# phymhan/pc-gan

Hardware: AMD Instinct MI355X
Metric: images/sec (G+D step) 128x128 bs32 per GPU (higher is better)
Workload: dtype f32; 1 GPU; wsgan_emb UTKFace-shaped 128x128 bs32/GPU fp32: 9-block ResnetGenerator + 3-layer PatchGAN + ResNet-18 Elo encoder@224 + AlexNet IP@224, full optimize_parameters(); global_batch=32, parallelism=dp1

## Files before the change

include/pcgan_hip.h:

```cpp
#ifndef PCGAN_HIP_H
#define PCGAN_HIP_H

#include <stddef.h>
#include <stdint.h>

#ifdef __cplusplus
extern "C" {
#endif

typedef void* pcgan_stream_t;

const char* pcgan_last_error(void);
int pcgan_version(void);
int pcgan_device_info(int* cu_count, char* arch, int arch_len);

typedef struct {
    int N, C, H, W;
    int K, R, S;
    int stride, pad, pad_mode;
    int P, Q;
    int dtype;
} pcgan_conv_desc;

enum { PCGAN_ACT_NONE = 0, PCGAN_ACT_RELU = 1, PCGAN_ACT_LRELU = 2, PCGAN_ACT_TANH = 3, PCGAN_ACT_SIGMOID = 4 };
// ... 203 lines not shown
    int stride, pad_h, pad_w;
    int P, Q;
    int k_off, K_total;
    int dtype;
} pcgan_iconv_desc;
int pcgan_iconv_supported(const pcgan_iconv_desc* d);
size_t pcgan_iconv_packed_bytes(const pcgan_iconv_desc* d);
int pcgan_iconv_pack(const pcgan_iconv_desc* d, int pool_expand, const float* w, const float* gamma, const float* beta, const float* mean,
                     const float* var, float eps, void* packed, pcgan_stream_t s);
int pcgan_iconv_fwd(const pcgan_iconv_desc* d, const void* x, const void* packed, void* y, int relu, pcgan_stream_t s);
int pcgan_maxpool_slice_fwd(const void* x, void* y, int N, int C, int H, int W, int k, int stride, int P, int Q, int k_off, int K_total,
                            int dtype, pcgan_stream_t s);
int pcgan_inception_prep(const void* x, void* y, int N, int C, int H, int W, int OH, int OW, const float* scale, const float* shift,
                         int dtype, pcgan_stream_t s);

int pcgan_linear_softmax_fwd(const void* x, const float* w, const float* b, void* logits, void* probs, int N, int C, int K, int dtype,
                             pcgan_stream_t s);

int pcgan_set_nonfinite_counter(unsigned int* dev_word);
int pcgan_set_option(const char* key, int value);
int pcgan_get_option(const char* key, int* value);
int pcgan_timer_enable(int capacity);
int pcgan_timer_read(int kind, float* ms, int cap);
#define PCGAN_IGEMM_LAUNCH_INFO 7
#define PCGAN_IGEMM_HGEMM_F16X2 1
#define PCGAN_IGEMM_HGEMM_BF16 2
#define PCGAN_IGEMM_IGEMM2_CG16 3
#define PCGAN_IGEMM_IGEMM2_CG4 4
#define PCGAN_IGEMM_GENERIC 5
#define PCGAN_IGEMM_SMALLM 6
int pcgan_igemm_last_launch(int* info, int n);

#ifdef __cplusplus
}
#endif
#endif
```

pc-gan_amd/csrc/capi.hip:

```cpp
#include "common.h"
#include <stdarg.h>
#include <atomic>
#include <mutex>
#include <vector>

namespace pcgan {
static thread_local char g_err[512] = "";
void set_error(const char* fmt, ...) {
    va_list ap;
    va_start(ap, fmt);
    vsnprintf(g_err, sizeof(g_err), fmt, ap);
    va_end(ap);
}
}

namespace pcgan {
namespace {
struct TimerKind {
    std::vector<hipEvent_t> start, stop;
    int used = 0;
};
std::mutex g_timer_mu;
std::atomic<int> g_timer_on{0};
TimerKind g_timer[TIMER_KINDS];
// ... 49 lines not shown
    }
    std::lock_guard<std::mutex> lk(g_timer_mu);
    TimerKind& t = g_timer[kind];
    int n = 0;
    for (int i = 0; i < t.used && n < cap; ++i) {
        if (hipEventSynchronize(t.stop[i]) != hipSuccess) continue;
        float v = 0.f;
        if (hipEventElapsedTime(&v, t.start[i], t.stop[i]) == hipSuccess) ms[n++] = v;
    }
    t.used = 0;
    return n;
}

namespace pcgan {
static std::atomic<unsigned*> g_nonfinite{nullptr};
unsigned* nonfinite_counter() { return g_nonfinite.load(std::memory_order_relaxed); }
}
extern "C" int pcgan_set_nonfinite_counter(unsigned int* dev_word) {
    pcgan::g_nonfinite.store(dev_word);
    return 0;
}

namespace pcgan {
static const char* const g_opt_names[OPT_COUNT] = {"bsplit_halo", "wgrad_gen", "wgrad_padcopy", "wgrad_cw", "hgemm_bf16", "wgd_look", "wgrad_direct", "hgemm_tile", "hgemm_ks", "wgrad_rowring"};
static std::atomic<int> g_opt[OPT_COUNT] = {{1}, {1}, {0}, {0}, {1}, {3}, {0}, {0}, {0}, {1}};
int option(int id) { return (id >= 0 && id < OPT_COUNT) ? g_opt[id].load(std::memory_order_relaxed) : 0; }
static int option_index(const char* key) {
    for (int i = 0; key && i < OPT_COUNT; ++i)
        if (strcmp(key, g_opt_names[i]) == 0) return i;
    return -1;
}
}
extern "C" int pcgan_set_option(const char* key, int value) {
    using namespace pcgan;
    const int i = option_index(key);
    PCGAN_CHECK(i >= 0, "set_option: unknown option '%s' (bsplit_halo, wgrad_gen, wgrad_padcopy, wgrad_cw, hgemm_bf16, wgd_look, wgrad_direct, hgemm_tile, hgemm_ks, wgrad_rowring)", key ? key : "(null)");
    PCGAN_CHECK(i != OPT_WGRAD_CW || value == 0 || value == 128 || value == 256, "set_option: wgrad_cw takes 0 (default), 128 or 256, got %d", value);
    PCGAN_CHECK(i != OPT_HGEMM_TILE || value == 0 || value == 128128 || value == 128064 || value == 64128 || value == 64064,
                "set_option: hgemm_tile takes 0 (heuristic) or BM * 1000 + BP with BM, BP in {64, 128}, got %d", value);
    PCGAN_CHECK(i != OPT_HGEMM_KS || (value >= 0 && value <= 8), "set_option: hgemm_ks takes 0 (heuristic) .. 8, got %d", value);
    g_opt[i].store(value);
    return 0;
}
extern "C" int pcgan_get_option(const char* key, int* value) {
    using namespace pcgan;
    const int i = option_index(key);
    PCGAN_CHECK(i >= 0 && value, "get_option: unknown option or null output");
    *value = g_opt[i].load();
    return 0;
}

extern "C" const char* pcgan_last_error(void) { return pcgan::g_err; }
extern "C" int pcgan_version(void) { return 100; }

extern "C" int pcgan_device_info(int* cu_count, char* arch, int arch_len) {
    hipDeviceProp_t prop;
    hipError_t e = hipGetDeviceProperties(&prop, 0);
    if (e != hipSuccess) {
        pcgan::set_error("hipGetDeviceProperties failed: %s", hipGetErrorString(e));
// ... 10 lines not shown
```

pc-gan_amd/csrc/common.h:

```cpp
#pragma once
#include <hip/hip_runtime.h>
#include <stdint.h>
#include <stdio.h>
#include <string.h>
#include "../../include/pcgan_hip.h"

namespace pcgan {

void set_error(const char* fmt, ...);

#define PCGAN_CHECK(cond, ...)                \
    do {                                      \
        if (!(cond)) {                        \
            pcgan::set_error(__VA_ARGS__);    \
            return 1;                         \
        }                                     \
    } while (0)

#define PCGAN_LAUNCH_CHECK()                                                      \
    do {                                                                          \
        hipError_t e__ = hipGetLastError();                                       \
        if (e__ != hipSuccess) {                                                  \
            pcgan::set_error("%s:%d launch failed: %s", __FILE__, __LINE__,       \
                             hipGetErrorString(e__));                             \
            return 2;                                                             \
        }                                                                         \
    } while (0)

enum { TIMER_RES_FWD = 0, TIMER_RES_DGRAD = 1, TIMER_RES_WGRAD = 2, TIMER_RES_WGRAD_MAIN = 3, TIMER_KINDS = 4 };
struct TimerScope {
    int kind, slot;
    hipStream_t st;
    TimerScope(int kind, hipStream_t st);
    ~TimerScope();
};

static inline int timer_kind_res(const pcgan_conv_desc* d, int kind) {
    return (d && d->K == 256 && d->C == 256 && d->R == 3 && d->S == 3 && d->stride == 1 && d->pad_mode == 1 && d->pad == 1) ? kind : -1;
}

enum { OPT_BSPLIT_HALO = 0, OPT_WGRAD_GEN = 1, OPT_WGRAD_PADCOPY = 2, OPT_WGRAD_CW = 3, OPT_HGEMM_BF16 = 4, OPT_WGD_LOOK = 5, OPT_WGRAD_DIRECT = 6, OPT_HGEMM_TILE = 7, OPT_HGEMM_KS = 8, OPT_WGRAD_ROWRING = 9, OPT_COUNT = 10 };
int option(int id);

unsigned* nonfinite_counter();
int launch_wgd_reduce(const float* part, float* dw, const float* scales, int splits, int K, int C, int accumulate, hipStream_t st);
__device__ __forceinline__ bool is_nonfinite(float v) { return (__float_as_uint(v) & 0x7f800000u) == 0x7f800000u; }
__device__ __forceinline__ void report_nonfinite(unsigned* counter, bool bad) {
    if (counter != nullptr && __builtin_amdgcn_ballot_w64(bad) != 0ull && (threadIdx.x & 63) == 0) atomicAdd(counter, 1u);
}

int launch_weight_row_absmax(const float* w, int K, int C, int T, int by_c, float* out, hipStream_t st);

int launch_reflect_fold(const void* padded, void* dx, int NC, int H, int W, int pad, int dtype, hipStream_t st);

static inline int ilog2_exact(int v) {
    int l = 0;
    while ((1 << l) < v) ++l;
    return ((1 << l) == v) ? l : -1;
}
static inline size_t align_up(size_t v, size_t a) { return (v + a - 1) / a * a; }

__device__ __forceinline__ float act_apply(float v, int act, float slope) {
    switch (act) {
        case PCGAN_ACT_RELU: return v > 0.f ? v : 0.f;
// ... 127 lines not shown
```

pc-gan_amd/csrc/hgemm.hip:

```cpp
#include "igemm.h"

namespace pcgan {

typedef _Float16 f16x8 __attribute__((ext_vector_type(8)));
typedef _Float16 f16x4 __attribute__((ext_vector_type(4)));

typedef __bf16 bf16x8v __attribute__((ext_vector_type(8)));
typedef __bf16 bf16x4v __attribute__((ext_vector_type(4)));

template <int MODE, int BM, int BP, typename TA>
__global__ void __launch_bounds__(256) hgemm_kernel(IgemmArgs a) {
    static_assert(MODE == MODE_FWD_ZERO || MODE == MODE_FWD_REFLECT || MODE == MODE_BWD, "forward and plain data gradient");
    constexpr bool HALF = sizeof(TA) == 2;
    constexpr int NP = HALF ? 1 : 2;
    constexpr unsigned ES = sizeof(TA);
    constexpr int WM = (BM == 128 || (BM == 64 && BP == 64)) ? 2 : 1;
    constexpr int WP = 4 / WM;
    constexpr int WMT = BM / WM, WPT = BP / WP;
    constexpr int MI = WMT / 32, PJ = WPT / 32;
    constexpr int KPT = BP / 16;
    constexpr int ACH = BM * 4 / 256;
    constexpr int TROWS = NTAP_FWD + 1;
    constexpr int AH = BM + 8;
    __shared__ __attribute__((aligned(16))) f16x8 As[2][NP][2 * AH];
    __shared__ __attribute__((aligned(16))) f16x8 Bs[2][NP][2 * BP];
    __shared__ unsigned offT[TROWS][BP];
    __shared__ __attribute__((aligned(16))) float biasS[BM];
    __shared__ __attribute__((aligned(16))) float iswS[BM];

    const int nMt = (a.M + BM - 1) / BM;
    const int mt = blockIdx.x % nMt;
    int pt = blockIdx.x / nMt;
    int phase = 0;
    while (phase + 1 < a.nphase && pt >= a.tstart[phase + 1]) ++phase;
    pt -= a.tstart[phase];
    const PhaseArgs& P = a.ph[phase];
    const int tid = threadIdx.x;
    const int lane = tid & 63, lo = lane & 31, hi = lane >> 5;
    const int wave = __builtin_amdgcn_readfirstlane(tid >> 6);
    const int wm = wave / WP, wp = wave % WP;
    const int Ptot = P.Ptot, Kp = P.Kp;
    const int m0 = mt * BM, p0 = pt * BP;
    const int ph_nS = P.nS;
    const int T = P.nR * ph_nS;
    const int HgWg4 = a.Hg * a.Wg * (int)ES;
    const __amdgpu_buffer_rsrc_t rX = make_rsrc(a.X, a.x_bytes);
    const __amdgpu_buffer_rsrc_t rA = make_rsrc(P.A, (unsigned)a.M * (unsigned)Kp * 4u);

    float sx = 1.f;
    const int pl = tid % BP;
    {
        const int pg = p0 + pl;
        const bool pvalid = pg < Ptot;
        int gn = 0, py = 0, px = 0;
        if (pvalid) pix_coord(a, P, pg, gn, py, px);
        const unsigned vbase = (unsigned)gn * (unsigned)a.Cg * (unsigned)(a.Hg * a.Wg);
        for (int t = tid / BP; t <= T; t += 256 / BP) {
            const int ri = t / ph_nS, sj = t - ri * ph_nS;
            const int r = P.r0 + ri * a.tstep, sxx = P.s0 + sj * a.tstep;
            const bool live = pvalid && t < T;
            const unsigned y = axis_entry<MODE>(py, py + a.pad, true, r, a.Hg, a.sl, a.pad);
            const unsigned x = axis_entry<MODE>(px, px + a.pad, true, sxx, a.Wg, a.sl, a.pad);
            offT[t][pl] = (live && y != 0xffffffffu && x != 0xffffffffu) ? (vbase + y * (unsigned)a.Wg + x) * ES : OOB;
        }
    }
    const int ksub = __builtin_amdgcn_readfirstlane(tid / BP);
    __syncthreads();

    const int nst_all = Kp >> 4;
    const int nst_per = a.ksplit > 1 ? (nst_all + a.ksplit - 1) / a.ksplit : nst_all;
    const int st_begin = a.ksplit > 1 ? (int)blockIdx.z * nst_per : 0;
    const int st_end = st_begin + nst_per < nst_all ? st_begin + nst_per : nst_all;
    const int nst_here = st_end > st_begin ? st_end - st_begin : 0;

    int it_tap, it_c, it_k0, it_left = nst_here;
    {
        const int cc0 = st_begin / T;
        it_tap = st_begin - cc0 * T;
        it_c = cc0 * 16;
        it_k0 = st_begin * 16;
    }
    unsigned a_base[ACH];
#pragma unroll
    for (int j = 0; j < ACH; ++j) {
        const int q = tid + 256 * j;
        const int row = q >> 2, kc = (q & 3) * 4;
        a_base[j] = (m0 + row < a.M) ? (unsigned)((m0 + row) * Kp + kc) * 4u : OOB;
    }
    struct Stage {
        u32x4 av[ACH];
        unsigned bv[KPT];
    };
    auto load = [&](Stage& r) {
        const bool live = it_left > 0;
        const unsigned vo = offT[live ? it_tap : T][pl];
        const unsigned so = (unsigned)((it_c + ksub * KPT) * HgWg4);
#pragma unroll
        for (int j = 0; j < ACH; ++j) r.av[j] = __builtin_amdgcn_raw_buffer_load_b128(rA, live ? a_base[j] : OOB, (unsigned)it_k0 * 4u, 0);
#pragma unroll
        for (int i = 0; i < KPT; ++i) {
            if constexpr (HALF) r.bv[i] = (unsigned)__builtin_amdgcn_raw_buffer_load_b16(rX, vo, so + (unsigned)(i * HgWg4), 0);
            else r.bv[i] = __builtin_amdgcn_raw_buffer_load_b32(rX, vo, so + (unsigned)(i * HgWg4), 0);
        }
        --it_left;
        const int t1 = it_tap + 1;
        const bool wr = t1 == T;
        it_tap = wr ? 0 : t1;
        it_c += wr ? 16 : 0;
        it_k0 += 16;
    };
    auto stash = [&](const Stage& r, int buf) {
        if constexpr (HALF) {
#pragma unroll
            for (int j = 0; j < ACH; ++j) {
                const int q = tid + 256 * j;
                const int row = q >> 2, kc = (q & 3) * 4;
                bf16x4v h;
#pragma unroll
                for (int e = 0; e < 4; ++e) h[e] = (__bf16)__uint_as_float(r.av[j][e]);
                *reinterpret_cast<bf16x4v*>(reinterpret_cast<__bf16*>(&As[buf][0][(kc >> 3) * AH + row]) + (kc & 4)) = h;
            }
            typedef unsigned short usK __attribute__((ext_vector_type(KPT)));
            usK v;
#pragma unroll
            for (int e = 0; e < KPT; ++e) v[e] = (unsigned short)r.bv[e];
            if constexpr (KPT == 8) *reinterpret_cast<usK*>(&Bs[buf][0][ksub * BP + pl]) = v;
            else *reinterpret_cast<usK*>(reinterpret_cast<unsigned short*>(&Bs[buf][0][(ksub >> 1) * BP + pl]) + (ksub & 1) * 4) = v;
            return;
        }
#pragma unroll
        for (int j = 0; j < ACH; ++j) {
            const int q = tid + 256 * j;
            const int row = q >> 2, kc = (q & 3) * 4;
            typedef unsigned u32x2 __attribute__((ext_vector_type(2)));
            u32x2 h, l;
            h[0] = r.av[j][0]; h[1] = r.av[j][1];
            l[0] = r.av[j][2]; l[1] = r.av[j][3];
            _Float16* d0 = reinterpret_cast<_Float16*>(&As[buf][0][(kc >> 3) * AH + row]) + (kc & 4);
            _Float16* d1 = reinterpret_cast<_Float16*>(&As[buf][NP - 1][(kc >> 3) * AH + row]) + (kc & 4);
            *reinterpret_cast<u32x2*>(d0) = h;
            *reinterpret_cast<u32x2*>(d1) = l;
        }
        if constexpr (KPT == 8) {
            f16x8 h, l;
#pragma unroll
            for (int e = 0; e < 8; ++e) {
                _Float16 x, y;
                split2h(__uint_as_float(r.bv[e]) * sx, x, y);
                h[e] = x;
                l[e] = y;
            }
            Bs[buf][0][ksub * BP + pl] = h;
            Bs[buf][NP - 1][ksub * BP + pl] = l;
        } else {
            f16x4 h, l;
#pragma unroll
            for (int e = 0; e < 4; ++e) {
                _Float16 x, y;
                split2h(__uint_as_float(r.bv[e]) * sx, x, y);
                h[e] = x;
                l[e] = y;
            }
            *reinterpret_cast<f16x4*>(reinterpret_cast<_Float16*>(&Bs[buf][0][(ksub >> 1) * BP + pl]) + (ksub & 1) * 4) = h;
            *reinterpret_cast<f16x4*>(reinterpret_cast<_Float16*>(&Bs[buf][NP - 1][(ksub >> 1) * BP + pl]) + (ksub & 1) * 4) = l;
        }
    };

    f32x16 acc[MI][PJ];
#pragma unroll
    for (int i = 0; i < MI; ++i)
#pragma unroll
        for (int j = 0; j < PJ; ++j)
#pragma unroll
            for (int r = 0; r < 16; ++r) acc[i][j][r] = 0.f;
    struct Operands {
        f16x8 A[NP][MI], B[NP][PJ];
    };
    auto fetch = [&](Operands& o, int buf) {
#pragma unroll
        for (int p = 0; p < NP; ++p) {
#pragma unroll
            for (int i = 0; i < MI; ++i) o.A[p][i] = As[buf][p][hi * AH + wm * WMT + i * 32 + lo];
#pragma unroll
            for (int j = 0; j < PJ; ++j) o.B[p][j] = Bs[buf][p][hi * BP + wp * WPT + j * 32 + lo];
        }
    };
    auto mma = [&](const Operands& o) {
        if constexpr (HALF) {
#pragma unroll
            for (int i = 0; i < MI; ++i)
#pragma unroll
                for (int j = 0; j < PJ; ++j)
                    acc[i][j] = __builtin_amdgcn_mfma_f32_32x32x16_bf16(__builtin_bit_cast(bf16x8v, o.A[0][i]), __builtin_bit_cast(bf16x8v, o.B[0][j]),
                                                                         acc[i][j], 0, 0, 0);
            return;
        }
        constexpr int PA[3] = {NP - 1, 0, 0}, PB[3] = {0, NP - 1, 0};
#pragma unroll
        for (int q = 0; q < 3; ++q)
#pragma unroll
            for (int i = 0; i < MI; ++i)
#pragma unroll
                for (int j = 0; j < PJ; ++j)
                    acc[i][j] = __builtin_amdgcn_mfma_f32_32x32x16_f16(o.A[PA[q]][i], o.B[PB[q]][j], acc[i][j], 0, 0, 0);
    };
    auto interleave = [&]() {
        constexpr int NM = (HALF ? 1 : 3) * MI * PJ, NRD = NP * (MI + PJ);
#pragma unroll
        for (int q = 0; q < NM; ++q) {
            __builtin_amdgcn_sched_group_barrier(0x008, 1, 0);
            __builtin_amdgcn_sched_group_barrier(0x100, (NRD + NM - 1) / NM, 0);
            __builtin_amdgcn_sched_group_barrier(0x002, 48 / NM + 1, 0);
            __builtin_amdgcn_sched_group_barrier(0x200, 1, 0);
            __builtin_amdgcn_sched_group_barrier(0x020, (ACH + KPT + NM - 1) / NM, 0);
        }
    };

    Stage rg[2];
    if (nst_here > 0) {
        load(rg[0]);
        load(rg[1]);
    }
    if constexpr (!HALF) {
        const float m = thread_max_of_partials(a.x_amax, a.x_namax, tid, 256);
        sx = pow2_scale(block_max(m, biasS));
        if (tid < BM) iswS[tid] = m0 + tid < a.M ? 1.f / pow2_scale(a.w_amax[m0 + tid]) : 1.f;
        __syncthreads();
    }
    if (tid < BM) biasS[tid] = (a.bias != nullptr && m0 + tid < a.M) ? a.bias[m0 + tid] : 0.f;
    if (nst_here == 0) __syncthreads();
    if (nst_here > 0) {
        Operands op[2];
        stash(rg[0], 0);
        __syncthreads();
        load(rg[0]);
        fetch(op[0], 0);
        stash(rg[1], 1);
        __syncthreads();
        load(rg[1]);
        const int nst2 = (nst_here + 1) & ~1;
        for (int s = 0; s < nst2; s += 2) {
#pragma unroll
            for (int t = 0; t < 2; ++t) {
                fetch(op[t ^ 1], t ^ 1);
                mma(op[t]);
                stash(rg[t], t);
                load(rg[t]);
                interleave();
                __builtin_amdgcn_sched_barrier(0);
                __syncthreads();
                __builtin_amdgcn_sched_barrier(0);
            }
        }
    }

    const float isx = 1.f / sx;
    const int YhYw = a.Yh * a.Yw;
    bool bad = false;
    if constexpr (!HALF) {
#pragma unroll
        for (int j = 0; j < PJ; ++j)
#pragma unroll
            for (int i = 0; i < MI; ++i)
#pragma unroll
                for (int r = 0; r < 16; ++r) bad |= is_nonfinite(acc[i][j][r]);
        report_nonfinite(a.ovf, bad);
    }
#pragma unroll
    for (int j = 0; j < PJ; ++j) {
        const int pix = p0 + wp * WPT + j * 32 + lo;
        if (pix >= Ptot) continue;
        int n, oy, ox;
// ... 1 lines not shown
        if (a.ksplit > 1) {
            float* Yp = a.Ypart + ((size_t)blockIdx.z * a.N + n) * a.M * YhYw + oy * a.Yw + ox;
#pragma unroll
            for (int i = 0; i < MI; ++i)
#pragma unroll
                for (int r = 0; r < 16; ++r) {
                    const int ml = wm * WMT + i * 32 + (r & 3) + 8 * (r >> 2) + 4 * hi;
                    const int m = m0 + ml;
                    if (m < a.M) Yp[(size_t)m * YhYw] = (acc[i][j][r] * isx) * (HALF ? 1.f : iswS[ml]);
                }
            continue;
        }
        TA* Yp = (TA*)a.Y + (size_t)n * a.M * YhYw + oy * a.Yw + ox;
#pragma unroll
        for (int i = 0; i < MI; ++i)
#pragma unroll
            for (int r = 0; r < 16; ++r) {
                const int ml = wm * WMT + i * 32 + (r & 3) + 8 * (r >> 2) + 4 * hi;
                if (m0 + ml < a.M) st1(Yp + (size_t)(m0 + ml) * YhYw, act_apply((acc[i][j][r] * isx) * (HALF ? 1.f : iswS[ml]) + biasS[ml], a.act, a.slope));
            }
    }
}

template <int MODE>
static void launch_mode(const IgemmArgs& a, int bm, int bp, dim3 grid2, hipStream_t st) {
    if (bm == 128 && bp == 128) LAUNCH_TA(a.dtype, hgemm_kernel, grid2, a, MODE, 128, 128);
    else if (bm == 128) LAUNCH_TA(a.dtype, hgemm_kernel, grid2, a, MODE, 128, 64);
    else if (bp == 128) LAUNCH_TA(a.dtype, hgemm_kernel, grid2, a, MODE, 64, 128);
    else LAUNCH_TA(a.dtype, hgemm_kernel, grid2, a, MODE, 64, 64);
}
int launch_hgemm(int mode, const IgemmArgs& a, int bm, int bp, dim3 grid2, hipStream_t st) {
    switch (mode) {
        case MODE_FWD_ZERO: launch_mode<MODE_FWD_ZERO>(a, bm, bp, grid2, st); break;
        case MODE_FWD_REFLECT: launch_mode<MODE_FWD_REFLECT>(a, bm, bp, grid2, st); break;
        case MODE_BWD: launch_mode<MODE_BWD>(a, bm, bp, grid2, st); break;
        default: PCGAN_CHECK(false, "hgemm: no kernel for mode %d", mode);
    }
    PCGAN_LAUNCH_CHECK();
    return 0;
}

}

using namespace pcgan;

__global__ void __launch_bounds__(256) hgemm_presplit_kernel(float* __restrict__ A, int M, int Kp4, const float* __restrict__ rowmax) {
    const size_t n4 = (size_t)M * Kp4;
    for (size_t i = (size_t)blockIdx.x * 256 + threadIdx.x; i < n4; i += (size_t)gridDim.x * 256) {
        const float s = pow2_scale(rowmax[i / Kp4]);
        const float4 v = reinterpret_cast<const float4*>(A)[i];
        f16x4 h, l;
        _Float16 x, y;
        split2h(v.x * s, x, y); h[0] = x; l[0] = y;
        split2h(v.y * s, x, y); h[1] = x; l[1] = y;
// ... 13 lines not shown
```

pc-gan_amd/csrc/igemm.h:

```cpp
#pragma once
#include "common.h"
#include <type_traits>

namespace pcgan {

typedef float f32x16 __attribute__((ext_vector_type(16)));

enum { MODE_FWD_ZERO = 0, MODE_FWD_REFLECT = 1, MODE_BWD = 2, MODE_BWD_REFLECT = 3 };

typedef unsigned int u32x4 __attribute__((ext_vector_type(4)));
static constexpr unsigned OOB = 0x80000000u;

__device__ __forceinline__ __amdgpu_buffer_rsrc_t make_rsrc(const void* p, unsigned bytes) {
    return __builtin_amdgcn_make_buffer_rsrc(const_cast<void*>(p), 0, (int)bytes, 0x00020000);
}
__device__ __forceinline__ float ld_b32(__amdgpu_buffer_rsrc_t r, unsigned voff, unsigned soff) {
    return __uint_as_float(__builtin_amdgcn_raw_buffer_load_b32(r, voff, soff, 0));
}
__device__ __forceinline__ float4 ld_b128(__amdgpu_buffer_rsrc_t r, unsigned voff) {
    const u32x4 v = __builtin_amdgcn_raw_buffer_load_b128(r, voff, 0, 0);
    return make_float4(__uint_as_float(v.x), __uint_as_float(v.y), __uint_as_float(v.z), __uint_as_float(v.w));
}

template <typename TA>
// ... 91 lines not shown

struct IgemmArgs {
    const void* X;
    void* Y;
    int dtype;
    const float* bias;
    int M, N, Cg, Cgp, Hg, Wg;
    int Yh, Yw;
    int ostep, sl, pad, tstep;
    int act;
    float slope;
    unsigned x_bytes;
    int nphase;
    int rowfold;
    int chunked;
    int ksplit;
    float* Ypart;
    int tstart[17];
    PhaseArgs ph[16];
    const float* x_amax;
    const float* w_amax;
    int x_namax, hsplit;
    unsigned* ovf;
};

struct Geom {
    int Hg, Wg, sl, pad;
};

template <int MODE>
__device__ __forceinline__ bool tap_offset(const Geom& a, int py, int px, int r, int s, int& off) {
    if (MODE == MODE_BWD || MODE == MODE_BWD_REFLECT) {
        const int ty = py + a.pad - r, tx = px + a.pad - s;
        const int oy = ty >> a.sl, ox = tx >> a.sl;
        off = oy * a.Wg + ox;
        return (ty >= 0) & (tx >= 0) & (oy < a.Hg) & (ox < a.Wg);
    } else {
        int iy = (py << a.sl) - a.pad + r;
        int ix = (px << a.sl) - a.pad + s;
        if (MODE == MODE_FWD_REFLECT) {
            iy = iy < 0 ? -iy : iy;
            iy = iy >= a.Hg ? 2 * (a.Hg - 1) - iy : iy;
            ix = ix < 0 ? -ix : ix;
            ix = ix >= a.Wg ? 2 * (a.Wg - 1) - ix : ix;
            off = iy * a.Wg + ix;
            return true;
        } else {
// ... 65 lines not shown
    int M, Kp, N, Cg, Cgp, Hg, Wg, Ho, Wo;
    int sl, pad, S;
    int magicS;
    int Ptot, chunks_per_split;
    unsigned x_bytes, dy_bytes;
};

static constexpr unsigned SM_INV = 0x40000000u;

static inline int round4(int v) { return (v + 3) & ~3; }
static inline size_t esz(const pcgan_conv_desc* d) { return d->dtype == PCGAN_BF16 ? 2 : 4; }

#define LAUNCH_TA(dt, KERNEL, GRID, ARG, ...)                                                                   \
    do {                                                                                                        \
        if ((dt) == PCGAN_BF16) hipLaunchKernelGGL((KERNEL<__VA_ARGS__, bf16>), GRID, dim3(256), 0, st, ARG);    \
        else hipLaunchKernelGGL((KERNEL<__VA_ARGS__, float>), GRID, dim3(256), 0, st, ARG);                      \
    } while (0)

static inline unsigned capped_blocks(size_t total, unsigned per_block, unsigned cap) {
    const size_t b = (total + per_block - 1) / per_block;
    return (unsigned)(b > cap ? cap : (b < 1 ? 1 : b));
}

void record_launch(int form, int mode, int bm, int bp, int ks, int nphase);
int launch_splitk_reduce(int dtype, hipStream_t st, const float* part, void* y, const float* bias, int ks, size_t out_elems, int M,
                         int HW, int act, float slope);

int launch_igemm_f32(int mode, const IgemmArgs& a, int bm, int bp, dim3 grid, dim3 grid2, hipStream_t st);
int launch_hgemm(int mode, const IgemmArgs& a, int bm, int bp, dim3 grid2, hipStream_t st);
int launch_hgemm_presplit(float* A, int M, int Kp4, const float* rowmax, hipStream_t st);
int launch_smallm(int mode, IgemmArgs& a, int pmax, hipStream_t st, float* part_ws, size_t part_bytes);
int launch_transpose4(const float* A, float* At, int M, int Kp, hipStream_t st);
int launch_pack_strip(const float* A, float* Ws, int M, int Cg, int Cgp, int nR, int nS, hipStream_t st);
int wgrad_splits(const pcgan_conv_desc* d, int* chunks_per_split);
int launch_wgrad(const pcgan_conv_desc* d, const WgradArgs& a, int splits, float* dw, int accumulate, hipStream_t st);

}
```

pc-gan_amd/csrc/igemm_conv.hip:

```cpp
#include "igemm.h"
#include <stdlib.h>
#include <mutex>

namespace pcgan {

template <typename TA>
__global__ void splitk_reduce_kernel(const float* __restrict__ part, TA* __restrict__ y, const float* __restrict__ bias,
                                     int ks, size_t n, int M, int HW, int act, float slope) {
    const size_t n4 = (n & 3) ? 0 : (n >> 2);
    const size_t stride = (size_t)gridDim.x * blockDim.x;
    for (size_t i = blockIdx.x * (size_t)blockDim.x + threadIdx.x; i < n4; i += stride) {
        float4 acc = reinterpret_cast<const float4*>(part)[i];
        for (int s = 1; s < ks; ++s) {
            const float4 v = reinterpret_cast<const float4*>(part + (size_t)s * n)[i];
            acc.x += v.x; acc.y += v.y; acc.z += v.z; acc.w += v.w;
        }
        float o[4] = {acc.x, acc.y, acc.z, acc.w};
#pragma unroll
        for (int u = 0; u < 4; ++u) {
            const size_t e = i * 4 + u;
            if (bias) o[u] += bias[(e / HW) % M];
            o[u] = act_apply(o[u], act, slope);
        }
        st4(y + 4 * i, make_float4(o[0], o[1], o[2], o[3]));
// ... 191 lines not shown
        *ks = k;
        return;
    }
    if (allow_split && may_split(M, ptot_max, nphase) && nst >= 32) {
        const long b = tile_blocks(M, ptot_max, nphase, m, 128);
        int k = (int)(512 / b);
        if (k > 8) k = 8;
        if (k > nst / 8) k = nst / 8;
        if (k >= 2) {
            *bm = m;
            *bp = 128;
            *ks = k;
            return;
        }
    }
    if (m >= 64 && tile_blocks(M, ptot_max, nphase, m, p) < 384) p = 64;
    if (m == 128 && tile_blocks(M, ptot_max, nphase, m, p) < 384) m = 64;
    *bm = m;
    *bp = p;
}

static std::mutex g_launch_mu;
static int g_launch[PCGAN_IGEMM_LAUNCH_INFO] = {0};
void record_launch(int form, int mode, int bm, int bp, int ks, int nphase) {
    std::lock_guard<std::mutex> lk(g_launch_mu);
    const int seq = g_launch[0] + 1;
    const int v[PCGAN_IGEMM_LAUNCH_INFO] = {seq, form, mode, bm, bp, ks, nphase};
    for (int i = 0; i < PCGAN_IGEMM_LAUNCH_INFO; ++i) g_launch[i] = v[i];
}

static int launch_igemm(int mode, IgemmArgs& a, hipStream_t st, float* part_ws = nullptr, size_t part_bytes = 0) {
    int pmax = 0;
    for (int i = 0; i < a.nphase; ++i) pmax = a.ph[i].Ptot > pmax ? a.ph[i].Ptot : pmax;
    if (pmax <= 0 || a.nphase <= 0) return 0;
    if (a.M <= 4) return launch_smallm(mode, a, pmax, st, part_ws, part_bytes);
    int bm, bp, ks;
    int nst_min = 1 << 30;
    for (int i = 0; i < a.nphase; ++i) nst_min = (a.ph[i].Kp + 15) / 16 < nst_min ? (a.ph[i].Kp + 15) / 16 : nst_min;
    const size_t out_elems = (size_t)a.N * a.M * a.Yh * a.Yw;
    choose_tile(a.M, pmax, a.nphase, nst_min, part_ws != nullptr, &bm, &bp, &ks);
    if (ks > 1 && (size_t)ks * out_elems * 4 > part_bytes) ks = 1;
    a.ksplit = ks;
    a.Ypart = part_ws;
    const dim3 grid((unsigned)(((a.M + bm - 1) / bm) * ((pmax + bp - 1) / bp)), (unsigned)a.nphase, (unsigned)ks);
    a.tstart[0] = 0;
    for (int i = 0; i < a.nphase; ++i) a.tstart[i + 1] = a.tstart[i] + (a.ph[i].Ptot + bp - 1) / bp;
    const dim3 grid2((unsigned)(((a.M + bm - 1) / bm) * a.tstart[a.nphase]), 1u, (unsigned)ks);
    const bool cg16 = a.chunked == 1, cg4 = a.chunked == 2;
    PCGAN_CHECK(cg16 || mode != MODE_BWD_REFLECT, "igemm: fused reflect data-gradient needs K %% 16 == 0");
    if (cg4) {
        PCGAN_CHECK(a.Cgp == 4, "igemm: 4-channel stages need a 3-/4-channel tensor");
        for (int i = 0; i < a.nphase; ++i)
            PCGAN_CHECK(a.ph[i].nR * a.ph[i].nS <= NTAP_CG4, "igemm: 4-channel stages: more than %d taps", NTAP_CG4);
    }
    if (cg16) {
        PCGAN_CHECK((a.Cg % 16) == 0, "igemm: chunked K order needs a multiple of 16 channels");
        for (int i = 0; i < a.nphase; ++i)
            PCGAN_CHECK(a.ph[i].nR * a.ph[i].nS <= (mode == MODE_BWD_REFLECT ? NTAP_MIR : NTAP_FWD) && (a.ph[i].Kp % 16) == 0,
                        "igemm: chunked K order: bad phase");
    }
    const bool half = a.dtype == PCGAN_BF16 && option(OPT_HGEMM_BF16) != 0;
    if ((half || (a.hsplit && a.dtype == PCGAN_F32)) && cg16 && mode != MODE_BWD_REFLECT && bm >= 64) {
        record_launch(half ? PCGAN_IGEMM_HGEMM_BF16 : PCGAN_IGEMM_HGEMM_F16X2, mode, bm, bp, ks, a.nphase);
        if (int e = launch_hgemm(mode, a, bm, bp, grid2, st)) return e;
    } else {
        record_launch(cg16 ? PCGAN_IGEMM_IGEMM2_CG16 : (cg4 ? PCGAN_IGEMM_IGEMM2_CG4 : PCGAN_IGEMM_GENERIC), mode, bm, bp, ks, a.nphase);
        if (int e = launch_igemm_f32(mode, a, bm, bp, grid, grid2, st)) return e;
    }
    if (ks > 1 && launch_splitk_reduce(a.dtype, st, part_ws, a.Y, a.bias, ks, out_elems, a.M, a.Yh * a.Yw, a.act, a.slope)) return 2;
    return 0;
}

}

using namespace pcgan;

static size_t fwd_part_bytes(const pcgan_conv_desc* d) {
    const int ptot = d->N * d->P * d->Q;
    if (d->K <= 4) return (ptot <= 65536 && d->C >= 64) ? align_up((size_t)8 * d->K * ptot * 4, 256) : 0;
    return may_split(d->K, ptot, 1) ? align_up((size_t)8 * d->N * d->K * d->P * d->Q * 4, 256) : 0;
}
static size_t bwd_part_bytes(const pcgan_conv_desc* d) {
    const int s = d->stride;
    const int pmax = d->N * ((d->H + s - 1) / s) * ((d->W + s - 1) / s);
    return may_split(d->C, pmax, s * s) ? align_up((size_t)8 * d->N * d->C * d->H * d->W * 4, 256) : 0;
}
// ... 362 lines not shown
```

pc-gan_amd/hip/lib.py:

```python
import ctypes
import os

_HERE = os.path.dirname(os.path.abspath(__file__))
LIB_PATH = os.environ.get('PCGAN_LIB') or os.path.join(os.path.dirname(_HERE), 'lib', 'libpcgan_hip.so')

ACT_NONE, ACT_RELU, ACT_LRELU, ACT_TANH, ACT_SIGMOID = 0, 1, 2, 3, 4
PASS_FWD, PASS_BWD_DATA, PASS_BWD_WEIGHT = 0, 1, 2
F32, BF16 = 0, 1


class ImageDesc(ctypes.Structure):
    _fields_ = [(n, ctypes.c_int) for n in ('H', 'W', 'RH', 'RW', 'FH', 'FW', 'ksize_h', 'ksize_v', 'out_channels')]


class ResBlockDesc(ctypes.Structure):
    _fields_ = [('N', ctypes.c_int), ('C', ctypes.c_int), ('H', ctypes.c_int), ('W', ctypes.c_int), ('eps', ctypes.c_float),
                ('momentum', ctypes.c_float), ('dtype', ctypes.c_int)]


class ConvDesc(ctypes.Structure):
    _fields_ = [(n, ctypes.c_int) for n in
                ('N', 'C', 'H', 'W', 'K', 'R', 'S', 'stride', 'pad', 'pad_mode', 'P', 'Q', 'dtype')]


# ... 130 lines not shown
    global _lib
    if _lib is not None:
        return _lib
    if not os.path.exists(LIB_PATH):
        raise RuntimeError(
            'pcgan_amd: %s not found -- build it with `python -c "import __graft_entry__ as g; g.build()"` '
            '(or `make -C pc-gan_amd/csrc`). There is no fallback path.' % LIB_PATH)
    import torch
    bundled = os.path.join(os.path.dirname(torch.__file__), 'lib', 'libamdhip64.so')
    if os.path.exists(bundled):
        ctypes.CDLL(bundled, mode=ctypes.RTLD_GLOBAL)
    lib = ctypes.CDLL(LIB_PATH)
    for name, (res, args) in SIGNATURES.items():
        fn = getattr(lib, name)
        fn.restype = res
        fn.argtypes = args
    _lib = lib
    _options_from_environment(lib)
    return lib


_ENV_OPTIONS = (('PCGAN_BSPLIT_HALO', 'bsplit_halo', int), ('PCGAN_WGRAD_GEN', 'wgrad_gen', int), ('PCGAN_WGRAD_PADCOPY', 'wgrad_padcopy', int),
                ('PCGAN_WGRAD_CW', 'wgrad_cw', int), ('PCGAN_HGEMM', 'hgemm_bf16', int), ('PCGAN_WGRAD_DIRECT', 'wgrad_direct', int),
                ('PCGAN_WGD_LOOK', 'wgd_look', int), ('PCGAN_WGRAD_ROWRING', 'wgrad_rowring', int))


def _options_from_environment(lib):
    for env, key, conv in _ENV_OPTIONS:
        v = os.environ.get(env)
        if v not in (None, ''):
            set_option(key, conv(v), lib)


def set_option(key, value, lib=None):
    lib = lib or load()
    if lib.pcgan_set_option(key.encode(), int(value)) != 0:
        msg = lib.pcgan_last_error()
        raise RuntimeError('pcgan_hip set_option failed: %s' % (msg.decode() if msg else '?'))


def get_option(key):
    v = ctypes.c_int(0)
    if load().pcgan_get_option(key.encode(), ctypes.byref(v)) != 0:
        raise RuntimeError('pcgan_hip get_option: unknown option %r' % key)
    return v.value


# ... 5 lines not shown
```

pc-gan_amd/hip/ops.py:

```python
import ctypes
import os

import torch

from . import lib as _L
from .lib import ConvDesc, ResBlockDesc, ACT_NONE, F32, BF16

_vp = ctypes.c_void_p


def _p(t):
    return _vp(t.data_ptr()) if t is not None else _vp(0)


_DEVICE_INDEX = []


def _raw_stream():
    if not _DEVICE_INDEX:
        _DEVICE_INDEX.append(torch.cuda.current_device())
    return torch._C._cuda_getCurrentRawStream(_DEVICE_INDEX[0])


def _stream():
# ... 787 lines not shown
    return dx


TIMER_KINDS = {'res_fwd': 0, 'res_dgrad': 1, 'res_wgrad': 2, 'res_wgrad_main': 3}


def timer_enable(capacity):
    _L.check(_L.load().pcgan_timer_enable(int(capacity)), 'timer_enable')


def timer_read(kind, cap=65536):
    buf = (ctypes.c_float * cap)()
    n = _L.load().pcgan_timer_read(TIMER_KINDS[kind], buf, cap)
    if n < 0:
        raise RuntimeError('pcgan_timer_read failed')
    return [float(buf[i]) for i in range(n)]


IGEMM_FORMS = {1: 'hgemm_f16x2', 2: 'hgemm_bf16', 3: 'igemm2_cg16', 4: 'igemm2_cg4', 5: 'igemm', 6: 'smallm'}
IGEMM_MODES = {0: 'fwd_zero', 1: 'fwd_reflect', 2: 'dgrad', 3: 'dgrad_reflect'}


def igemm_last_launch():
    buf = (ctypes.c_int * 7)()
    _L.check(_L.load().pcgan_igemm_last_launch(buf, 7), 'igemm_last_launch')
    seq, form, mode, bm, bp, ks, nph = list(buf)
    return {'seq': seq, 'form': IGEMM_FORMS.get(form), 'mode': IGEMM_MODES.get(mode), 'bm': bm, 'bp': bp, 'ks': ks, 'nphase': nph}


def channel_sum(x, accumulate_into=None):
    _chk(accumulate_into)
    dt = _act(x)
    N, C = x.shape[0], x.shape[1]
    HW = x.numel() // (N * C)
    out = accumulate_into if accumulate_into is not None else torch.empty(C, dtype=torch.float32, device=x.device)
    psum = getattr(x, '_pcgan_plane_sums', None)
    if psum is not None and psum.numel() == N * C and psum.device == x.device:
        PLANE_SUM_STATS['fused'] += 1
        if getattr(x, '_pcgan_plane_sums_stream', None) != _raw_stream():
            psum.record_stream(torch.cuda.current_stream())
        _L.check(_L.load().pcgan_sum_planes(_p(psum), _p(out), N, C, int(accumulate_into is not None), _stream()), 'sum_planes')
        return out
    PLANE_SUM_STATS['full'] += 1
    scratch = torch.empty(N * C, dtype=torch.float32, device=x.device)
    _L.check(_L.load().pcgan_channel_sum(_p(x), _p(out), _p(scratch), N, C, HW, int(accumulate_into is not None), dt,
                                         _stream()), 'channel_sum')
    return out


def act_fwd(x, act, slope=0.0):
# ... 349 lines not shown
```

Measured before the change: 1217 images/sec.

## Add shared-memory input window form to fp32 split-half hgemm conv kernel

```diff
diff --git a/include/pcgan_hip.h b/include/pcgan_hip.h
--- a/include/pcgan_hip.h
+++ b/include/pcgan_hip.h
@@ -249,7 +249,8 @@
 int pcgan_get_option(const char* key, int* value);
 int pcgan_timer_enable(int capacity);
 int pcgan_timer_read(int kind, float* ms, int cap);
-#define PCGAN_IGEMM_LAUNCH_INFO 7
+#define PCGAN_IGEMM_LAUNCH_INFO 10
+#define PCGAN_IGEMM_LAUNCH_WIN 9
 #define PCGAN_IGEMM_HGEMM_F16X2 1
 #define PCGAN_IGEMM_HGEMM_BF16 2
 #define PCGAN_IGEMM_IGEMM2_CG16 3
diff --git a/pc-gan_amd/csrc/capi.hip b/pc-gan_amd/csrc/capi.hip
--- a/pc-gan_amd/csrc/capi.hip
+++ b/pc-gan_amd/csrc/capi.hip
@@ -95,8 +95,8 @@
 }
 
 namespace pcgan {
-static const char* const g_opt_names[OPT_COUNT] = {"bsplit_halo", "wgrad_gen", "wgrad_padcopy", "wgrad_cw", "hgemm_bf16", "wgd_look", "wgrad_direct", "hgemm_tile", "hgemm_ks", "wgrad_rowring"};
-static std::atomic<int> g_opt[OPT_COUNT] = {{1}, {1}, {0}, {0}, {1}, {3}, {0}, {0}, {0}, {1}};
+static const char* const g_opt_names[OPT_COUNT] = {"bsplit_halo", "wgrad_gen", "wgrad_padcopy", "wgrad_cw", "hgemm_bf16", "wgd_look", "wgrad_direct", "hgemm_tile", "hgemm_ks", "wgrad_rowring", "hgemm_window"};
+static std::atomic<int> g_opt[OPT_COUNT] = {{1}, {1}, {0}, {0}, {1}, {3}, {0}, {0}, {0}, {1}, {1}};
 int option(int id) { return (id >= 0 && id < OPT_COUNT) ? g_opt[id].load(std::memory_order_relaxed) : 0; }
 static int option_index(const char* key) {
     for (int i = 0; key && i < OPT_COUNT; ++i)
@@ -107,7 +107,7 @@
 extern "C" int pcgan_set_option(const char* key, int value) {
     using namespace pcgan;
     const int i = option_index(key);
-    PCGAN_CHECK(i >= 0, "set_option: unknown option '%s' (bsplit_halo, wgrad_gen, wgrad_padcopy, wgrad_cw, hgemm_bf16, wgd_look, wgrad_direct, hgemm_tile, hgemm_ks, wgrad_rowring)", key ? key : "(null)");
+    PCGAN_CHECK(i >= 0, "set_option: unknown option '%s' (bsplit_halo, wgrad_gen, wgrad_padcopy, wgrad_cw, hgemm_bf16, wgd_look, wgrad_direct, hgemm_tile, hgemm_ks, wgrad_rowring, hgemm_window)", key ? key : "(null)");
     PCGAN_CHECK(i != OPT_WGRAD_CW || value == 0 || value == 128 || value == 256, "set_option: wgrad_cw takes 0 (default), 128 or 256, got %d", value);
     PCGAN_CHECK(i != OPT_HGEMM_TILE || value == 0 || value == 128128 || value == 128064 || value == 64128 || value == 64064,
                 "set_option: hgemm_tile takes 0 (heuristic) or BM * 1000 + BP with BM, BP in {64, 128}, got %d", value);
diff --git a/pc-gan_amd/csrc/common.h b/pc-gan_amd/csrc/common.h
--- a/pc-gan_amd/csrc/common.h
+++ b/pc-gan_amd/csrc/common.h
@@ -39,7 +39,7 @@
     return (d && d->K == 256 && d->C == 256 && d->R == 3 && d->S == 3 && d->stride == 1 && d->pad_mode == 1 && d->pad == 1) ? kind : -1;
 }
 
-enum { OPT_BSPLIT_HALO = 0, OPT_WGRAD_GEN = 1, OPT_WGRAD_PADCOPY = 2, OPT_WGRAD_CW = 3, OPT_HGEMM_BF16 = 4, OPT_WGD_LOOK = 5, OPT_WGRAD_DIRECT = 6, OPT_HGEMM_TILE = 7, OPT_HGEMM_KS = 8, OPT_WGRAD_ROWRING = 9, OPT_COUNT = 10 };
+enum { OPT_BSPLIT_HALO = 0, OPT_WGRAD_GEN = 1, OPT_WGRAD_PADCOPY = 2, OPT_WGRAD_CW = 3, OPT_HGEMM_BF16 = 4, OPT_WGD_LOOK = 5, OPT_WGRAD_DIRECT = 6, OPT_HGEMM_TILE = 7, OPT_HGEMM_KS = 8, OPT_WGRAD_ROWRING = 9, OPT_HGEMM_WINDOW = 10, OPT_COUNT = 11 };
 int option(int id);
 
 unsigned* nonfinite_counter();
diff --git a/pc-gan_amd/csrc/hgemm.hip b/pc-gan_amd/csrc/hgemm.hip
--- a/pc-gan_amd/csrc/hgemm.hip
+++ b/pc-gan_amd/csrc/hgemm.hip
@@ -8,9 +8,11 @@
 typedef __bf16 bf16x8v __attribute__((ext_vector_type(8)));
 typedef __bf16 bf16x4v __attribute__((ext_vector_type(4)));
 
-template <int MODE, int BM, int BP, typename TA>
+
+template <int MODE, int BM, int BP, typename TA, bool WIN = false>
 __global__ void __launch_bounds__(256) hgemm_kernel(IgemmArgs a) {
     static_assert(MODE == MODE_FWD_ZERO || MODE == MODE_FWD_REFLECT || MODE == MODE_BWD, "forward and plain data gradient");
+    static_assert(!WIN || (sizeof(TA) == 4 && MODE != MODE_FWD_REFLECT), "window form: fp32 tensors, zero padding");
     constexpr bool HALF = sizeof(TA) == 2;
     constexpr int NP = HALF ? 1 : 2;
     constexpr unsigned ES = sizeof(TA);
@@ -21,10 +23,12 @@
     constexpr int KPT = BP / 16;
     constexpr int ACH = BM * 4 / 256;
     constexpr int TROWS = NTAP_FWD + 1;
+    constexpr int WIN_ITEMS = win_items(BM, BP);
     constexpr int AH = BM + 8;
     __shared__ __attribute__((aligned(16))) f16x8 As[2][NP][2 * AH];
-    __shared__ __attribute__((aligned(16))) f16x8 Bs[2][NP][2 * BP];
-    __shared__ unsigned offT[TROWS][BP];
+    __shared__ __attribute__((aligned(16))) f16x8 Bs[WIN ? 1 : 2][NP][WIN ? 1 : 2 * BP];
+    __shared__ unsigned offT[WIN ? 1 : TROWS][BP];
+    extern __shared__ __attribute__((aligned(16))) f16x8 Wn[];
     __shared__ __attribute__((aligned(16))) float biasS[BM];
     __shared__ __attribute__((aligned(16))) float iswS[BM];
 
@@ -49,7 +53,35 @@
 
     float sx = 1.f;
     const int pl = tid % BP;
-    {
+    const int NPA = a.win_npos + 1;
+    unsigned wvo[WIN_ITEMS], wrec[WIN_ITEMS], wbase[PJ];
+    if constexpr (WIN) {
+        const int pitch = a.win_pitch, Hq = a.Hg + a.win_g;
+        auto flat = [&](int pix) {
+            int n, py, px;
+            pix_coord(a, P, pix, n, py, px);
+            return (n * Hq + a.win_g + py - a.win_padT) * pitch + a.win_gx + px - a.win_padL;
+        };
+        const int fmin = flat(p0);
+#pragma unroll
+        for (int j = 0; j < PJ; ++j) {
+            const int pix = p0 + wp * WPT + j * 32 + lo;
+            wbase[j] = pix < Ptot ? (unsigned)(flat(pix) - fmin) : 0u;
+        }
+#pragma unroll
+        for (int j = 0; j < WIN_ITEMS; ++j) {
+            const int idx = tid + 256 * j;
+            const int kh = idx >= a.win_npos ? 1 : 0;
+            const int pos = idx - kh * a.win_npos;
+            const bool idle = pos >= a.win_npos;
+            const int f = fmin + pos;
+            const int V = f / pitch, cx = f - V * pitch;
+            const int n = V / Hq, vy = V - n * Hq;
+            const bool ok = !idle && cx >= a.win_gx && vy >= a.win_g && n < a.N;
+            wvo[j] = ok ? (unsigned)(((n * a.Cg + kh * 8) * a.Hg + (vy - a.win_g)) * a.Wg + (cx - a.win_gx)) * ES : OOB;
+            wrec[j] = idle ? (unsigned)a.win_npos : (unsigned)(kh * NPA + pos);
+        }
+    } else {
         const int pg = p0 + pl;
         const bool pvalid = pg < Ptot;
         int gn = 0, py = 0, px = 0;
@@ -65,7 +97,7 @@
         }
     }
     const int ksub = __builtin_amdgcn_readfirstlane(tid / BP);
-    __syncthreads();
+    if constexpr (!WIN) __syncthreads();
 
     const int nst_all = Kp >> 4;
     const int nst_per = a.ksplit > 1 ? (nst_all + a.ksplit - 1) / a.ksplit : nst_all;
@@ -73,10 +105,11 @@
     const int st_end = st_begin + nst_per < nst_all ? st_begin + nst_per : nst_all;
     const int nst_here = st_end > st_begin ? st_end - st_begin : 0;
 
-    int it_tap, it_c, it_k0, it_left = nst_here;
+    int it_tap, it_c, it_k0, it_left = nst_here, it_tap0 = 0;
     {
         const int cc0 = st_begin / T;
         it_tap = st_begin - cc0 * T;
+        it_tap0 = it_tap;
         it_c = cc0 * 16;
         it_k0 = st_begin * 16;
     }
@@ -98,7 +131,7 @@
 #pragma unroll
         for (int j = 0; j < ACH; ++j) r.av[j] = __builtin_amdgcn_raw_buffer_load_b128(rA, live ? a_base[j] : OOB, (unsigned)it_k0 * 4u, 0);
 #pragma unroll
-        for (int i = 0; i < KPT; ++i) {
+        for (int i = 0; i < (WIN ? 0 : KPT); ++i) {
             if constexpr (HALF) r.bv[i] = (unsigned)__builtin_amdgcn_raw_buffer_load_b16(rX, vo, so + (unsigned)(i * HgWg4), 0);
             else r.bv[i] = __builtin_amdgcn_raw_buffer_load_b32(rX, vo, so + (unsigned)(i * HgWg4), 0);
         }
@@ -141,7 +174,8 @@
             *reinterpret_cast<u32x2*>(d0) = h;
             *reinterpret_cast<u32x2*>(d1) = l;
         }
-        if constexpr (KPT == 8) {
+        if constexpr (WIN) {
+        } else if constexpr (KPT == 8) {
             f16x8 h, l;
 #pragma unroll
             for (int e = 0; e < 8; ++e) {
@@ -176,7 +210,54 @@
     struct Operands {
         f16x8 A[NP][MI], B[NP][PJ];
     };
+    const int wT = T;
+    int f_ri = 0, f_sj = 0, f_buf = 0, f_left = nst_here;
+    int w_c = 0, w_buf = 0;
+    unsigned wv[WIN_ITEMS][8];
+    auto wload = [&]() {
+        const bool live = (w_c >> 4) * wT < st_end;
+#pragma unroll
+        for (int j = 0; j < WIN_ITEMS; ++j)
+#pragma unroll
+            for (int i = 0; i < 8; ++i)
+                wv[j][i] = __builtin_amdgcn_raw_buffer_load_b32(rX, live ? wvo[j] : OOB, (unsigned)((w_c + i) * HgWg4), 0);
+        w_c += 16;
+    };
+    auto wstash = [&]() {
+#pragma unroll
+        for (int j = 0; j < WIN_ITEMS; ++j) {
+            f16x8 h, l;
+#pragma unroll
+            for (int e = 0; e < 8; ++e) {
+                _Float16 x, y;
+                split2h(__uint_as_float(wv[j][e]) * sx, x, y);
+                h[e] = x;
+                l[e] = y;
+            }
+            Wn[(w_buf * NP + 0) * 2 * NPA + wrec[j]] = h;
+            Wn[(w_buf * NP + NP - 1) * 2 * NPA + wrec[j]] = l;
+        }
+        w_buf ^= 1;
+    };
     auto fetch = [&](Operands& o, int buf) {
+        if constexpr (WIN) {
+            const int sh = MODE == MODE_BWD ? (P.nR - 1 - f_ri) * a.win_pitch + (ph_nS - 1 - f_sj) : f_ri * a.win_pitch + f_sj;
+#pragma unroll
+            for (int p = 0; p < NP; ++p) {
+#pragma unroll
+                for (int i = 0; i < MI; ++i) o.A[p][i] = As[buf][p][hi * AH + wm * WMT + i * 32 + lo];
+#pragma unroll
+                for (int j = 0; j < PJ; ++j) o.B[p][j] = Wn[((f_buf * NP + p) * 2 + hi) * NPA + sh + wbase[j]];
+            }
+            const bool adv = f_left > 1;
+            --f_left;
+            const bool ws = f_sj + 1 == ph_nS;
+            const bool wt = ws && f_ri + 1 == P.nR;
+            f_sj = adv ? (ws ? 0 : f_sj + 1) : f_sj;
+            f_ri = adv ? (wt ? 0 : (ws ? f_ri + 1 : f_ri)) : f_ri;
+            f_buf ^= (adv && wt) ? 1 : 0;
+            return;
+        }
 #pragma unroll
         for (int p = 0; p < NP; ++p) {
 #pragma unroll
@@ -220,6 +301,12 @@
     if (nst_here > 0) {
         load(rg[0]);
         load(rg[1]);
+        if constexpr (WIN) {
+            f_ri = it_tap0 / ph_nS;
+            f_sj = it_tap0 - f_ri * ph_nS;
+            w_c = (st_begin / T) * 16;
+            wload();
+        }
     }
     if constexpr (!HALF) {
         const float m = thread_max_of_partials(a.x_amax, a.x_namax, tid, 256);
@@ -231,6 +318,14 @@
     if (nst_here == 0) __syncthreads();
     if (nst_here > 0) {
         Operands op[2];
+        if constexpr (WIN) {
+            wstash();
+            wload();
+            if (it_tap0 == T - 1) {
+                wstash();
+                wload();
+            }
+        }
         stash(rg[0], 0);
         __syncthreads();
         load(rg[0]);
@@ -245,9 +340,17 @@
                 fetch(op[t ^ 1], t ^ 1);
                 mma(op[t]);
                 stash(rg[t], t);
+                bool wdue = false;
+                if constexpr (WIN) wdue = it_tap == 2 && it_left > -2;
                 load(rg[t]);
                 interleave();
                 __builtin_amdgcn_sched_barrier(0);
+                if constexpr (WIN) {
+                    if (wdue) {
+                        wstash();
+                        wload();
+                    }
+                }
                 __syncthreads();
                 __builtin_amdgcn_sched_barrier(0);
             }
@@ -295,14 +398,27 @@
     }
 }
 
+#define LAUNCH_WIN(GRID, ARG, LDS, ...) hipLaunchKernelGGL((hgemm_kernel<__VA_ARGS__, float, true>), GRID, dim3(256), LDS, st, ARG)
 template <int MODE>
 static void launch_mode(const IgemmArgs& a, int bm, int bp, dim3 grid2, hipStream_t st) {
+    if constexpr (MODE != MODE_FWD_REFLECT) {
+        if (a.win_npos > 0) {
+            const size_t wlds = hgemm_window_lds(a.win_npos);
+            if (bm == 128 && bp == 128) LAUNCH_WIN(grid2, a, wlds, MODE, 128, 128);
+            else if (bm == 128) LAUNCH_WIN(grid2, a, wlds, MODE, 128, 64);
+            else if (bp == 128) LAUNCH_WIN(grid2, a, wlds, MODE, 64, 128);
+            else LAUNCH_WIN(grid2, a, wlds, MODE, 64, 64);
+            return;
+        }
+    }
     if (bm == 128 && bp == 128) LAUNCH_TA(a.dtype, hgemm_kernel, grid2, a, MODE, 128, 128);
     else if (bm == 128) LAUNCH_TA(a.dtype, hgemm_kernel, grid2, a, MODE, 128, 64);
     else if (bp == 128) LAUNCH_TA(a.dtype, hgemm_kernel, grid2, a, MODE, 64, 128);
     else LAUNCH_TA(a.dtype, hgemm_kernel, grid2, a, MODE, 64, 64);
 }
 int launch_hgemm(int mode, const IgemmArgs& a, int bm, int bp, dim3 grid2, hipStream_t st) {
+    PCGAN_CHECK(a.win_npos == 0 || (mode != MODE_FWD_REFLECT && a.dtype == PCGAN_F32 && a.win_npos <= 128 * win_items(bm, bp)),
+                "hgemm: window form asked for an unsupported launch");
     switch (mode) {
         case MODE_FWD_ZERO: launch_mode<MODE_FWD_ZERO>(a, bm, bp, grid2, st); break;
         case MODE_FWD_REFLECT: launch_mode<MODE_FWD_REFLECT>(a, bm, bp, grid2, st); break;
diff --git a/pc-gan_amd/csrc/igemm.h b/pc-gan_amd/csrc/igemm.h
--- a/pc-gan_amd/csrc/igemm.h
+++ b/pc-gan_amd/csrc/igemm.h
@@ -137,7 +137,10 @@
     const float* w_amax;
     int x_namax, hsplit;
     unsigned* ovf;
-};
+    int win_npos, win_pitch, win_g, win_gx, win_padT, win_padL;
+};
+static constexpr int win_items(int bm, int bp) { return bm == 128 && bp == 128 ? 2 : 3; }
+static inline size_t hgemm_window_lds(int npos) { return (size_t)128 * (size_t)(npos + 1); }
 
 struct Geom {
     int Hg, Wg, sl, pad;
@@ -249,7 +252,7 @@
     return (unsigned)(b > cap ? cap : (b < 1 ? 1 : b));
 }
 
-void record_launch(int form, int mode, int bm, int bp, int ks, int nphase);
+void record_launch(int form, int mode, int bm, int bp, int ks, int nphase, int win = 0);
 int launch_splitk_reduce(int dtype, hipStream_t st, const float* part, void* y, const float* bias, int ks, size_t out_elems, int M,
                          int HW, int act, float slope);
 
diff --git a/pc-gan_amd/csrc/igemm_conv.hip b/pc-gan_amd/csrc/igemm_conv.hip
--- a/pc-gan_amd/csrc/igemm_conv.hip
+++ b/pc-gan_amd/csrc/igemm_conv.hip
@@ -237,11 +237,34 @@
 
 static std::mutex g_launch_mu;
 static int g_launch[PCGAN_IGEMM_LAUNCH_INFO] = {0};
-void record_launch(int form, int mode, int bm, int bp, int ks, int nphase) {
+void record_launch(int form, int mode, int bm, int bp, int ks, int nphase, int win) {
     std::lock_guard<std::mutex> lk(g_launch_mu);
     const int seq = g_launch[0] + 1;
-    const int v[PCGAN_IGEMM_LAUNCH_INFO] = {seq, form, mode, bm, bp, ks, nphase};
+    const int v[PCGAN_IGEMM_LAUNCH_INFO] = {seq, form, mode, bm, bp, ks, nphase, 0, 0, win};
     for (int i = 0; i < PCGAN_IGEMM_LAUNCH_INFO; ++i) g_launch[i] = v[i];
+}
+
+static bool window_plan(int mode, IgemmArgs& a, int bm, int bp) {
+    a.win_npos = 0;
+    if (!option(OPT_HGEMM_WINDOW) || a.dtype != PCGAN_F32 || (mode != MODE_FWD_ZERO && mode != MODE_BWD)) return false;
+    if (a.nphase != 1 || a.sl != 0 || a.ostep != 1 || a.tstep != 1 || a.ph[0].ymap) return false;
+    const PhaseArgs& p = a.ph[0];
+    const int nR = p.nR, nS = p.nS;
+    if (nR * nS < 4 || nR * nS > NTAP_FWD || p.Hs != a.Yh || p.Ws != a.Yw || p.fy || p.fx || p.r0 || p.s0) return false;
+    const int padT = mode == MODE_BWD ? nR - 1 - a.pad : a.pad, padL = mode == MODE_BWD ? nS - 1 - a.pad : a.pad;
+    if (padT < 0 || padL < 0 || padT > nR - 1 || padL > nS - 1) return false;
+    const int padB = a.Yh + nR - 2 - padT - (a.Hg - 1), padR = a.Yw + nS - 2 - padL - (a.Wg - 1);
+    const int g = padT > padB ? padT : (padB > 0 ? padB : 0), gx = padL > padR ? padL : (padR > 0 ? padR : 0);
+    const int pitch = a.Wg + gx, ew = pitch - a.Yw, eh = a.Hg + g - a.Yh;
+    if (ew < 0 || eh < 0) return false;
+    const long wraps = (bp - 2) / a.Yw + 1, cross = (bp - 2) / (a.Yh * a.Yw) + 1;
+    const long npos = (bp - 1) + wraps * ew + cross * eh * pitch + (long)(nR - 1) * pitch + (nS - 1) + 1;
+    const long lds_static = 128L * (bm + 8) + 8L * bm + 4L * bp + 64;
+    if (npos > 128 * win_items(bm, bp) || (long)hgemm_window_lds((int)npos) + lds_static > 65536) return false;
+    if ((long)a.N * (a.Hg + g) * pitch + npos >= (1L << 30)) return false;
+    if (npos * 4 > (long)nR * nS * bp) return false;
+    a.win_npos = (int)npos; a.win_pitch = pitch; a.win_g = g; a.win_gx = gx; a.win_padT = padT; a.win_padL = padL;
+    return true;
 }
 
 static int launch_igemm(int mode, IgemmArgs& a, hipStream_t st, float* part_ws = nullptr, size_t part_bytes = 0) {
@@ -276,7 +299,8 @@
     }
     const bool half = a.dtype == PCGAN_BF16 && option(OPT_HGEMM_BF16) != 0;
     if ((half || (a.hsplit && a.dtype == PCGAN_F32)) && cg16 && mode != MODE_BWD_REFLECT && bm >= 64) {
-        record_launch(half ? PCGAN_IGEMM_HGEMM_BF16 : PCGAN_IGEMM_HGEMM_F16X2, mode, bm, bp, ks, a.nphase);
+        const bool win = window_plan(mode, a, bm, bp);
+        record_launch(half ? PCGAN_IGEMM_HGEMM_BF16 : PCGAN_IGEMM_HGEMM_F16X2, mode, bm, bp, ks, a.nphase, win ? 1 : 0);
         if (int e = launch_hgemm(mode, a, bm, bp, grid2, st)) return e;
     } else {
         record_launch(cg16 ? PCGAN_IGEMM_IGEMM2_CG16 : (cg4 ? PCGAN_IGEMM_IGEMM2_CG4 : PCGAN_IGEMM_GENERIC), mode, bm, bp, ks, a.nphase);
diff --git a/pc-gan_amd/hip/lib.py b/pc-gan_amd/hip/lib.py
--- a/pc-gan_amd/hip/lib.py
+++ b/pc-gan_amd/hip/lib.py
@@ -176,7 +176,8 @@
 
 _ENV_OPTIONS = (('PCGAN_BSPLIT_HALO', 'bsplit_halo', int), ('PCGAN_WGRAD_GEN', 'wgrad_gen', int), ('PCGAN_WGRAD_PADCOPY', 'wgrad_padcopy', int),
                 ('PCGAN_WGRAD_CW', 'wgrad_cw', int), ('PCGAN_HGEMM', 'hgemm_bf16', int), ('PCGAN_WGRAD_DIRECT', 'wgrad_direct', int),
-                ('PCGAN_WGD_LOOK', 'wgd_look', int), ('PCGAN_WGRAD_ROWRING', 'wgrad_rowring', int))
+                ('PCGAN_WGD_LOOK', 'wgd_look', int), ('PCGAN_WGRAD_ROWRING', 'wgrad_rowring', int),
+                ('PCGAN_HGEMM_WINDOW', 'hgemm_window', int))
 
 
 def _options_from_environment(lib):
diff --git a/pc-gan_amd/hip/ops.py b/pc-gan_amd/hip/ops.py
--- a/pc-gan_amd/hip/ops.py
+++ b/pc-gan_amd/hip/ops.py
@@ -833,10 +833,11 @@
 
 
 def igemm_last_launch():
-    buf = (ctypes.c_int * 7)()
-    _L.check(_L.load().pcgan_igemm_last_launch(buf, 7), 'igemm_last_launch')
-    seq, form, mode, bm, bp, ks, nph = list(buf)
-    return {'seq': seq, 'form': IGEMM_FORMS.get(form), 'mode': IGEMM_MODES.get(mode), 'bm': bm, 'bp': bp, 'ks': ks, 'nphase': nph}
+    buf = (ctypes.c_int * 10)()
+    _L.check(_L.load().pcgan_igemm_last_launch(buf, 10), 'igemm_last_launch')
+    seq, form, mode, bm, bp, ks, nph = list(buf)[:7]
+    return {'seq': seq, 'form': IGEMM_FORMS.get(form), 'mode': IGEMM_MODES.get(mode), 'bm': bm, 'bp': bp, 'ks': ks, 'nphase': nph,
+            'win': buf[9]}
 
 
 def channel_sum(x, accumulate_into=None):
```

Result: no change. 1228 images/sec, median of 6 (+0.9%).
